# ydchen0806/CLC

Measured on AMD Instinct MI355X. Metric: images/sec fwd+bwd @256x256 bs8; bpp+PSNR parity vs ref, higher is better.
Workload: dtype f32; 1 GPU; CLC N=64 lambda=0.0067 MSE, 256x256 bs8/GPU, n_refs=1: fwd + RD loss + bwd + clip_grad_norm + AdamW + aux step (configs[1]); global_batch=8, parallelism=dp1, ranks_seen=1, collective=none, hip_graph=True

## Files before the change

### clc_amd/csrc/conv_wgrad.hip

```cpp
#include "common.h"

#include <type_traits>

namespace {

constexpr int BK = 32;

constexpr unsigned kOOB = 0x80000000u;

__device__ __forceinline__ f32x4 buf_load4(__amdgpu_buffer_rsrc_t rsrc, unsigned byte_off) {
  return __builtin_bit_cast(f32x4, __builtin_amdgcn_raw_buffer_load_b128(rsrc, byte_off, 0, 0));
}

__device__ __forceinline__ int pin_s(int x) {
  int r;
  asm("s_mov_b32 %0, %1" : "=s"(r) : "s"(x));
  return r;
}

__device__ __forceinline__ void dma16(__amdgpu_buffer_rsrc_t rsrc, float* lds_dst, unsigned byte_off) {
#if defined(__HIP_DEVICE_COMPILE__)
  __builtin_amdgcn_raw_ptr_buffer_load_lds(rsrc, (__attribute__((address_space(3))) void*)lds_dst, 16, byte_off, 0, 0, 0);
#endif
}

struct WgradParams {
  const float* x; const float* dy; float* partial; float* bias_partial;
  unsigned x_bytes, dy_bytes;
  const float* dys; int lddys, dys_act, dys_pre; unsigned dys_bytes;
  int ow_shift, img_shift;
  int rmw;
  int N, H, W, Cin, ldx;
  int OH, OW, Cout, lddy;
  int ks, stride, pad, in_op;
  int K;
  int k_per_split;
  int nci;
};

struct OutSpec { float* w; float* b; int mode; };
typedef __bf16 bf16x8 __attribute__((ext_vector_type(8)));
__device__ __forceinline__ void split3(const float (&v)[8], bf16x8& h, bf16x8& m, bf16x8& l) {
#pragma unroll
  for (int e = 0; e < 8; ++e) {
    const __bf16 hb = (__bf16)v[e];
    const float r = v[e] - (float)hb;
    const __bf16 mb = (__bf16)r;
    const float r2 = r - (float)mb;
    h[e] = hb; m[e] = mb; l[e] = (__bf16)r2;
  }
}
#define MFMA_BF(a, b, c) __builtin_amdgcn_mfma_f32_32x32x16_bf16((a), (b), (c), 0, 0, 0)
#define MFMA_SPLIT6(ah, am, al, bh, bm, bl, c) do { \
    c = MFMA_BF(al, bh, c); c = MFMA_BF(ah, bl, c); c = MFMA_BF(am, bm, c); \
    c = MFMA_BF(am, bh, c); c = MFMA_BF(ah, bm, c); c = MFMA_BF(ah, bh, c); } while (0)

template <int BM, int BN, int WM, int WN, bool DMA = false, int BF = 0>
__device__ __forceinline__ void wgrad_body(const WgradParams& p, const int bx, const int by, const int k_begin, const int k_end, const OutSpec o, const int tid) {
  constexpr int NT = 64 * WM * WN;
  constexpr int TM = BM / WM / 32, TN = BN / WN / 32;
  constexpr int A_P = (BK * BM / 4 + NT - 1) / NT, B_P = (BK * BN / 4 + NT - 1) / NT;
  constexpr int AQ = BM / 4, BQ = BN / 4;
  extern __shared__ __attribute__((aligned(16))) float smem[];
  float* As = smem;
  float* Bs = smem + 2 * BK * BM;

  const int lane = tid & 63, wave = tid >> 6;
  const int wm = wave / WN, wn = wave % WN;
  const int tap = bx / p.nci, ci0 = (bx % p.nci) * BN;
  const int kh = tap / p.ks, kw = tap - kh * p.ks;
  const int co0 = by * BM;
  const int ntiles = (k_end - k_begin + BK - 1) / BK;
  const bool do_bias = (o.b != nullptr) && (bx == 0);
  const int pCout = pin_s(p.Cout), pCin = pin_s(p.Cin), pH = pin_s(p.H), pW = pin_s(p.W), pOH = pin_s(p.OH), pOW = pin_s(p.OW);
  const int plddy = pin_s(p.lddy), plddys = pin_s(p.lddys), pldx = pin_s(p.ldx), pstride = pin_s(p.stride), ppad = pin_s(p.pad);
  const int pows = pin_s(p.ow_shift), pimgs = pin_s(p.img_shift), pact = pin_s(p.dys_act), ppre = pin_s(p.dys_pre);

  f32x4 a_reg[A_P], b_reg[B_P], bias_acc[A_P], s_reg[A_P];
#pragma unroll
  for (int i = 0; i < A_P; ++i) bias_acc[i] = (f32x4){0.f, 0.f, 0.f, 0.f};

  const __amdgpu_buffer_rsrc_t xr = __builtin_amdgcn_make_buffer_rsrc(const_cast<float*>(p.x), 0, p.x_bytes, 0x00020000);
  const __amdgpu_buffer_rsrc_t dr = __builtin_amdgcn_make_buffer_rsrc(const_cast<float*>(p.dy), 0, p.dy_bytes, 0x00020000);
  const bool sq = p.in_op == CLC_IN_SQUARE;
  const bool fuse_act = p.dys != nullptr;
  const __amdgpu_buffer_rsrc_t sr = __builtin_amdgcn_make_buffer_rsrc(const_cast<float*>(fuse_act ? p.dys : p.dy), 0, fuse_act ? p.dys_bytes : p.dy_bytes, 0x00020000);
  auto load_tile = [&](int kt) {
    const int kbase = k_begin + kt * BK;
#pragma unroll
    for (int i = 0; i < A_P; ++i) {
      const int piece = tid + i * NT, row = piece / AQ, q = piece - row * AQ;
      const int pix = kbase + row, co = co0 + q * 4;
      const bool ok = row < BK && pix < k_end && co < pCout;
      a_reg[i] = buf_load4(dr, ok ? ((unsigned)pix * (unsigned)plddy + (unsigned)co) * 4u : kOOB);
      if (fuse_act) s_reg[i] = buf_load4(sr, ok ? ((unsigned)pix * (unsigned)plddys + (unsigned)co) * 4u : kOOB);
    }
#pragma unroll
    for (int i = 0; i < B_P; ++i) {
      const int piece = tid + i * NT, row = piece / BQ, q = piece - row * BQ;
      const int pix = kbase + row, ci = ci0 + q * 4;
      const int pp = pix < k_end ? pix : k_begin;
      int n, oy, ox;
      if (pows >= 0) {
        n = pp >> pimgs;
        const int r = pp & ((1 << pimgs) - 1);
        oy = r >> pows; ox = r & ((1 << pows) - 1);
      } else {
        n = pp / (pOH * pOW);
        const int r = pp - n * (pOH * pOW);
        oy = r / pOW; ox = r - oy * pOW;
      }
      const int iy = oy * pstride - ppad + kh, ix = ox * pstride - ppad + kw;
      const bool ok = row < BK && pix < k_end && ci < pCin && (unsigned)iy < (unsigned)pH && (unsigned)ix < (unsigned)pW;
      b_reg[i] = buf_load4(xr, ok ? ((unsigned)((n * pH + iy) * pW + ix) * (unsigned)pldx + (unsigned)ci) * 4u : kOOB);
    }
  };
  static_assert(!DMA || ((BK * BM / 4) % NT == 0 && (BK * BN / 4) % NT == 0), "whole DMA instructions per tile");
  constexpr bool use_dma = DMA;
  const int wave_base = (tid >> 6) * 64;
  auto dma_tile = [&](int kt, int buf) {
    const int kbase = k_begin + kt * BK;
#pragma unroll
    for (int i = 0; i < A_P; ++i) {
      const int piece = tid + i * NT, row = piece / AQ, q = piece - row * AQ;
      const int pix = kbase + row, co = co0 + q * 4;
      const bool ok = pix < k_end && co < pCout;
      dma16(dr, As + buf * BK * BM + (i * NT + wave_base) * 4, ok ? ((unsigned)pix * (unsigned)plddy + (unsigned)co) * 4u : kOOB);
    }
#pragma unroll
    for (int i = 0; i < B_P; ++i) {
      const int piece = tid + i * NT, row = piece / BQ, q = piece - row * BQ;
      const int pix = kbase + row, ci = ci0 + q * 4;
      const int pp = pix < k_end ? pix : k_begin;
      int n, oy, ox;
      if (pows >= 0) {
        n = pp >> pimgs;
        const int r = pp & ((1 << pimgs) - 1);
        oy = r >> pows; ox = r & ((1 << pows) - 1);
      } else {
        n = pp / (pOH * pOW);
        const int r = pp - n * (pOH * pOW);
// ... 537 lines not shown
  long unit_end[kMaxGroup];
  int T[kMaxGroup];
  int gx[kMaxGroup], gy[kMaxGroup];
  float* slots;
  int* plan;
  WgradParams p[kMaxGroup];
};

struct SKSeg { int idx, tile, k0, k1; };
__device__ __forceinline__ int sk_tid() {
  int t = threadIdx.x;
  asm volatile("" : "+v"(t));
  return t;
}
__device__ __forceinline__ int sk_find(const SKGroup& g, long u, int lo) {
  int hi = g.count - 1;
  while (lo < hi) {
    const int mid = (lo + hi) >> 1;
    if (u >= g.unit_end[mid]) lo = mid + 1; else hi = mid;
  }
  return lo;
}
__device__ __forceinline__ SKSeg sk_locate(const SKGroup& g, long u, long end, int& idx) {
  idx = sk_find(g, u, idx);
  const long base = idx ? g.unit_end[idx - 1] : 0;
  const int T = g.T[idx];
  const long local = u - base;
  SKSeg sgm;
  sgm.idx = idx;
  sgm.tile = (int)(local / T);
  sgm.k0 = (int)(local - (long)sgm.tile * T);
  const long k1 = (long)sgm.k0 + (end - u);
  sgm.k1 = k1 < T ? (int)k1 : T;
  return sgm;
}
__device__ __forceinline__ void sk_write_plan(const SKGroup& g, int w, long u0, long end) {
  if (threadIdx.x != 0) return;
  int idx = 0;
  const SKSeg sgm = sk_locate(g, u0, end, idx);
  int e0 = 0, e1 = 0, e2 = 0, e3 = 0;
  if (sgm.k0 > 0 && sgm.k1 == g.T[sgm.idx]) {
    const long ts = u0 - sgm.k0;
    long wf = ts * g.G / g.total;
    while ((wf + 1) * g.total / g.G <= ts) ++wf;
    while (wf * g.total / g.G > ts) --wf;
    e0 = sgm.idx; e1 = sgm.tile; e2 = (int)wf; e3 = 1;
  }
  int* dst = g.plan + 4 * w;
  dst[0] = e0; dst[1] = e1; dst[2] = e2; dst[3] = e3;
}

__device__ __forceinline__ OutSpec sk_out(const SKGroup& g, const WgradParams& p, const SKSeg& sgm, int T, int w, int tile_floats) {
  OutSpec o;
  if (sgm.k0 == 0 && sgm.k1 == T) {
    o.w = p.partial; o.b = p.bias_partial; o.mode = p.rmw ? 1 : 0;
  } else {
    float* slot = g.slots + ((size_t)w * 2 + (sgm.k0 > 0 ? 0 : 1)) * g.slot_floats;
    o.w = slot; o.b = p.bias_partial ? slot + tile_floats : nullptr; o.mode = 2;
  }
  return o;
}

template <int TW, bool DMA, int BF = 0>
__global__ __launch_bounds__(256, 2)
void conv_wgrad_taps_sk_kernel(const SKGroup g) {
  const int w = blockIdx.x;
  long u = (long)w * g.total / g.G;
  const long end = (long)(w + 1) * g.total / g.G;
  sk_write_plan(g, w, u, end);
  int idx = 0;
  bool first = true;
#pragma clang loop unroll(disable)
  while (u < end) {
    const SKSeg sgm = sk_locate(g, u, end, idx);
    const WgradParams& p = g.p[sgm.idx];
    const int gx = g.gx[sgm.idx];
    if (!first) __syncthreads();
    wgrad_taps_body<TW, DMA, BF>(p, sgm.tile % gx, sgm.tile / gx, sgm.k0, sgm.k1, sk_out(g, p, sgm, g.T[sgm.idx], w, 64 * 9 * 64), sk_tid());
    first = false;
    u += sgm.k1 - sgm.k0;
  }
}

constexpr int sk_wg_per_cu(int bm, int bn) { return bm * bn >= 128 * 128 ? 2 : (bm * bn >= 128 * 64 ? 3 : 5); }

template <int BM, int BN, int WM, int WN, bool DMA, int BF = 0>
__global__ __launch_bounds__(64 * WM * WN, (BM * BN >= 128 * 128 ? 2 : (BM * BN >= 128 * 64 ? 4 : 6)))
void conv_wgrad_sk_kernel(const SKGroup g) {
  const int w = blockIdx.x;
  long u = (long)w * g.total / g.G;
  const long end = (long)(w + 1) * g.total / g.G;
  sk_write_plan(g, w, u, end);
  int idx = 0;
  bool first = true;
#pragma clang loop unroll(disable)
  while (u < end) {
    const SKSeg sgm = sk_locate(g, u, end, idx);
    const WgradParams& p = g.p[sgm.idx];
    const int gx = g.gx[sgm.idx];
    if (!first) __syncthreads();
    const int ke = sgm.k1 * BK;
    wgrad_body<BM, BN, WM, WN, DMA, BF>(p, sgm.tile % gx, sgm.tile / gx, sgm.k0 * BK, ke < p.K ? ke : p.K, sk_out(g, p, sgm, g.T[sgm.idx], w, BM * BN), sk_tid());
    first = false;
    u += sgm.k1 - sgm.k0;
  }
}

constexpr int kFixY = 64;
template <int BM, int BN, int TAPS>
__global__ __launch_bounds__(256) void wgrad_sk_fixup_kernel(const SKGroup g) {
  constexpr int TILE = BM * TAPS * BN;
  __shared__ f32x4 sm[4][64];
  __shared__ int list[1280];
  __shared__ int wave_cnt[4];
  const int tid = threadIdx.x;
  int n_list = 0;
  {
    const int lane = tid & 63, wv = tid >> 6;
    for (int base = 0; base < g.G; base += 256) {
      const int w = base + tid;
      const bool on = w < g.G && g.plan[4 * w + 3] != 0;
      const unsigned long long m = __ballot(on);
      if (lane == 0) wave_cnt[wv] = __popcll(m);
      __syncthreads();
      int off = n_list, tot = 0;
      for (int q = 0; q < 4; ++q) { if (q < wv) off += wave_cnt[q]; tot += wave_cnt[q]; }
      if (on) list[off + __popcll(m & ((1ull << lane) - 1ull))] = w;
      n_list += tot;
      __syncthreads();
    }
  }
  const int col = tid & 63, grp = tid >> 6;
  const int e = (blockIdx.x * 64 + col) * 4;
  for (int li = blockIdx.y; li < n_list; li += kFixY) {
    const int wl = list[li];
    const int idx = g.plan[4 * wl], tile = g.plan[4 * wl + 1], wf = g.plan[4 * wl + 2];
    const WgradParams& p = g.p[idx];
    const int gx = g.gx[idx];
    const int bx = tile % gx, by = tile / gx;
    const bool is_bias = e >= TILE;
    const bool live = e < TILE + BM && !(is_bias && !(p.bias_partial && bx == 0));
    f32x4 s = {0.f, 0.f, 0.f, 0.f};
    if (live) {
      const int n = wl - wf + 1;
      auto src = [&](int i) { return reinterpret_cast<const f32x4*>(g.slots + ((size_t)(wf + i) * 2 + (i == 0 ? 1 : 0)) * g.slot_floats + e); };
      int i = grp;
      for (; i + 12 < n; i += 16) {
        const f32x4 a0 = *src(i), a1 = *src(i + 4), a2 = *src(i + 8), a3 = *src(i + 12);
        s += a0; s += a1; s += a2; s += a3;
      }
      for (; i < n; i += 4) s += *src(i);
    }
    __syncthreads();
    sm[grp][col] = s;
    __syncthreads();
    if (grp != 0 || !live) continue;
    s = (sm[0][col] + sm[1][col]) + (sm[2][col] + sm[3][col]);
    const int co0 = by * BM;
    if (is_bias) {
      const int c = e - TILE;
#pragma unroll
      for (int q = 0; q < 4; ++q)
        if (co0 + c + q < p.Cout) { float* dst = p.bias_partial + co0 + c + q; *dst = (p.rmw ? *dst : 0.f) + s[q]; }
      continue;
    }
    int cl, tap, cil, ci0, T9;
    if (TAPS == 9) { cl = e / (9 * BN); const int r = e - cl * 9 * BN; tap = r / BN; cil = r - tap * BN; ci0 = bx * BN; T9 = 9; }
    else { cl = e / BN; cil = e - cl * BN; tap = bx / p.nci; ci0 = (bx - tap * p.nci) * BN; T9 = p.ks * p.ks; }
    const int co = co0 + cl, ci = ci0 + cil;
    if (co >= p.Cout || ci >= p.Cin) continue;
    f32x4* dst = reinterpret_cast<f32x4*>(p.partial + ((size_t)co * T9 + tap) * p.Cin + ci);
// ... 65 lines not shown
      const int k = e >> 7, c = e & 127, pix = kb + k;
      float gv = (pix < k_end && co0 + c < p.Cout) ? p.dy[(size_t)pix * p.lddy + co0 + c] : 0.f;
      if (p.dys && pix < k_end && co0 + c < p.Cout) gv *= act_deriv(p.dys[(size_t)pix * p.lddys + co0 + c], p.dys_act, p.dys_pre);
      dyS[k][c] = gv;
    }
    for (int e = tid; e < 32 * 32; e += 256) {
      const int k = e >> 5, j = e & 31, pix = kb + k;
      float v = 0.f;
      if (pix < k_end && j < ncol) {
        const int tap = j / p.Cin, ci = j - tap * p.Cin, kh = tap / p.ks, kw = tap - kh * p.ks;
        const int n = pix / (p.OH * p.OW), r = pix - n * (p.OH * p.OW);
        const int oy = r / p.OW, ox = r - oy * p.OW;
        const int iy = oy * p.stride - p.pad + kh, ix = ox * p.stride - p.pad + kw;
        if (iy >= 0 && ix >= 0 && iy < p.H && ix < p.W) {
          v = p.x[(size_t)((n * p.H + iy) * p.W + ix) * p.ldx + ci];
          if (p.in_op == CLC_IN_SQUARE) v *= v;
        }
      }
      xS[k][j] = v;
    }
    __syncthreads();
#pragma unroll 4
    for (int k = 0; k < 32; ++k) {
      const float g = dyS[k][co_l];
      bsum += g;
#pragma unroll
      for (int j = 0; j < 16; ++j) acc[j] = fmaf(g, xS[k][jh * 16 + j], acc[j]);
    }
  }
  if (co < p.Cout) {
#pragma unroll
    for (int j = 0; j < 16; ++j)
      if (jh * 16 + j < ncol) {
        float* dst = p.partial + ((size_t)split * p.Cout + co) * ncol + jh * 16 + j;
        *dst = p.rmw ? *dst + acc[j] : acc[j];
      }
    if (jh == 0 && p.bias_partial) {
      float* dst = p.bias_partial + (size_t)split * p.Cout + co;
      *dst = p.rmw ? *dst + bsum : bsum;
    }
  }
}

struct Plan { int bm, bn, splits, k_per_split, nci; bool small; int taps; };

Plan make_plan(const clc_wgrad_desc* d) {
  Plan pl;
  pl.taps = 0;
  const long K = (long)d->N * d->OH * d->OW;
  const int T = d->ks * d->ks;
  pl.small = !((d->Cin % 4 == 0) && (d->ldx % 4 == 0) && (d->Cout % 4 == 0) && (d->lddy % 4 == 0));
  if (pl.small) {
    pl.bm = pl.bn = 0; pl.nci = 1;
    int splits = (int)((K + 255) / 256);
    if (splits < 1) splits = 1;
    if (splits > 512) splits = 512;
    long kps = (K + splits - 1) / splits;
    pl.k_per_split = (int)kps; pl.splits = (int)((K + kps - 1) / kps);
    return pl;
  }
  {
    auto lg = [](int v) { int s = 0; while ((1 << s) < v) ++s; return (1 << s) == v ? s : -1; };
    const int la = lg(d->OW), lb = lg(d->OH * d->OW), tw = d->OW < 32 ? d->OW : 32;
    const bool eligible = d->ks == 3 && d->stride == 1 && d->pad == 1 && la >= 3 && lb >= 0 && d->OH >= 32 / tw;
    if (eligible) {
      pl.taps = tw; pl.bm = 64; pl.bn = 64; pl.nci = (d->Cin + 63) / 64;
      const long ktiles = K / 32, tiles = (long)((d->Cout + 63) / 64) * pl.nci;
      long sp = (ktiles + 15) / 16;
      const long fill = (256 + tiles - 1) / tiles;
      if (sp < fill) sp = fill;
      if (sp > ktiles / 2) sp = ktiles / 2 > 0 ? ktiles / 2 : 1;
      const long cap = 512 / tiles > 0 ? 512 / tiles : 1;
      if (sp > cap) sp = cap;
      const long kt = (ktiles + sp - 1) / sp;
      pl.k_per_split = (int)(kt * 32);
      pl.splits = (int)((ktiles + kt - 1) / kt);
      return pl;
    }
  }
  const int bms[2] = {128, 64}, bns[2] = {128, 64};
  const long wsz = (long)d->Cout * T * d->Cin;
  long best_cost = -1, splits = 1;
  pl.bm = 64; pl.bn = 64;
  for (int a = 0; a < 2; ++a)
    for (int b = 0; b < 2; ++b) {
      const int bm = bms[a], bn = bns[b];
      if (bm == 128 && d->Cout < 128) continue;
      if (bn == 128 && (d->Cin < 128 || d->Cin % 128 != 0)) continue;
      const long tiles = (long)((d->Cout + bm - 1) / bm) * ((d->Cin + bn - 1) / bn) * T;
      const long eff_pct = (bm == 128 && bn == 128) ? 100 : ((bm == 128 || bn == 128) ? 80 : 55);
      const long mfma_per_ktile = (long)(bm / 32) * (bn / 32) / 4 * 16 * 64 * 100 / eff_pct;
      const long max_sp = K / 64 > 0 ? K / 64 : 1;
      for (long sp = 1; sp <= 256 && sp <= max_sp; ++sp) {
        const long ktiles = (K / sp + BK - 1) / BK;
        const long chain = ktiles * mfma_per_ktile + 6000;
        const long rounds = (tiles * sp + 255) / 256;
        const long slab = sp > 1 ? 12000 + sp * wsz / 200 : 0;
        const long cost = rounds * chain + slab;
        if (best_cost < 0 || cost < best_cost) { best_cost = cost; pl.bm = bm; pl.bn = bn; splits = sp; }
      }
    }
  pl.nci = (d->Cin + pl.bn - 1) / pl.bn;
  long kps = (K + splits - 1) / splits;
  kps = (kps + BK - 1) / BK * BK;
  pl.k_per_split = (int)kps;
  pl.splits = (int)((K + kps - 1) / kps);
  return pl;
}

}

extern "C" size_t clc_conv2d_wgrad_workspace_bytes(const clc_wgrad_desc* d) {
  if (!d) return 0;
  if (d->ks == 5) return clc_conv5_wgrad_workspace_bytes(d);
  Plan pl = make_plan(d);
  const size_t wsz = (size_t)d->Cout * d->ks * d->ks * d->Cin;
  return ((size_t)pl.splits * (wsz + d->Cout) + 64) * sizeof(float);
}

namespace {

int prepare(const clc_wgrad_desc* d, Plan& pl, WgradParams& p, bool sk = false) {
  CLC_CHECK(d && d->x && d->dy && d->dw, "clc_conv2d_wgrad: null pointer");
  CLC_CHECK(d->ks == 1 || d->ks == 3, "clc_conv2d_wgrad: ks must be 1 or 3 here (ks = 5 problems are launched in line by clc_conv2d_wgrad, never grouped)");
  CLC_CHECK(d->stride == 1 || d->stride == 2, "clc_conv2d_wgrad: stride must be 1 or 2");
  CLC_CHECK(d->OH == (d->H + 2 * d->pad - d->ks) / d->stride + 1 && d->OW == (d->W + 2 * d->pad - d->ks) / d->stride + 1,
            "clc_conv2d_wgrad: output dims inconsistent");
  CLC_CHECK(d->ldx >= d->Cin && d->lddy >= d->Cout, "clc_conv2d_wgrad: ld too small");
  CLC_CHECK((long)d->N * d->H * d->W < (1l << 31) && (long)d->N * d->OH * d->OW < (1l << 31), "clc_conv2d_wgrad: too many pixels");
  pl = make_plan(d);
  if (!(sk && clc_tuning[CLC_TUNE_WGRAD_STREAMK] && !pl.small))
    CLC_CHECK(d->workspace && d->workspace_bytes >= clc_conv2d_wgrad_workspace_bytes(d), "clc_conv2d_wgrad: workspace too small");
  const int T = d->ks * d->ks;
  const size_t wsz = (size_t)d->Cout * T * d->Cin;
  p.x = d->x; p.dy = d->dy;
  const bool direct = (pl.splits == 1);
  p.rmw = direct && d->accumulate;
  p.partial = direct ? d->dw : (float*)d->workspace;
  p.bias_partial = d->dbias ? (direct ? d->dbias : (float*)d->workspace + (size_t)pl.splits * wsz) : nullptr;
  p.N = d->N; p.H = d->H; p.W = d->W; p.Cin = d->Cin; p.ldx = d->ldx;
  p.OH = d->OH; p.OW = d->OW; p.Cout = d->Cout; p.lddy = d->lddy;
  p.ks = d->ks; p.stride = d->stride; p.pad = d->pad; p.in_op = d->in_op;
  p.K = d->N * d->OH * d->OW; p.k_per_split = pl.k_per_split; p.nci = pl.nci;
  const size_t xb = ((size_t)d->N * d->H * d->W - 1) * d->ldx * 4 + (size_t)d->Cin * 4;
  const size_t db = ((size_t)d->N * d->OH * d->OW - 1) * d->lddy * 4 + (size_t)d->Cout * 4;
  CLC_CHECK(xb < (1ull << 31) && db < (1ull << 31), "clc_conv2d_wgrad: tensor larger than 2 GiB");
  p.x_bytes = (unsigned)xb; p.dy_bytes = (unsigned)db;
  auto lg = [](int v) { int s = 0; while ((1 << s) < v) ++s; return (1 << s) == v ? s : -1; };
  const int la = lg(d->OW), lb = lg(d->OH * d->OW);
  p.ow_shift = (la >= 0 && lb >= 0) ? la : -1; p.img_shift = (la >= 0 && lb >= 0) ? lb : -1;
  p.dys = d->dys; p.lddys = d->lddys; p.dys_act = d->dys_act; p.dys_pre = d->dys_pre; p.dys_bytes = 0;
  if (d->dys) {
    CLC_CHECK(d->lddys >= d->Cout, "clc_conv2d_wgrad: bad dys");
    const size_t sb = ((size_t)d->N * d->OH * d->OW - 1) * d->lddys * 4 + (size_t)d->Cout * 4;
    CLC_CHECK(sb < (1ull << 31), "clc_conv2d_wgrad: dys larger than 2 GiB");
    p.dys_bytes = (unsigned)sb;
  }
  if (pl.small) CLC_CHECK(T * d->Cin <= 32, "clc_conv2d_wgrad: small/unaligned path needs ks*ks*Cin <= 32 (got %d)", T * d->Cin);
  else CLC_CHECK(aligned16(d->x) && aligned16(d->dy), "clc_conv2d_wgrad: unaligned pointers");
  return 0;
}

struct Pending { const clc_wgrad_desc* d; Plan pl; WgradParams p; };

template <int BM, int BN>
int launch_variant(const Pending* pend, int n, hipStream_t st) {
  WgradGroup g;
  g.count = 0;
  int total = 0;
  for (int i = 0; i < n; ++i) {
    const Pending& e = pend[i];
    if (e.pl.small || e.pl.taps || e.pl.bm != BM || e.pl.bn != BN) continue;
    const int T = e.d->ks * e.d->ks;
    const int gx = e.pl.nci * T, gy = (e.d->Cout + BM - 1) / BM;
    total += gx * gy * e.pl.splits;
    g.gx[g.count] = gx; g.gy[g.count] = gy; g.wg_end[g.count] = total; g.p[g.count] = e.p;
    ++g.count;
  }
  if (g.count == 0) return 0;
  const size_t lds = (size_t)2 * BK * (BM + BN) * sizeof(float);
  if (g.count == 1) {
    const int last = g.wg_end[0] / (g.gx[0] * g.gy[0]);
    hipLaunchKernelGGL((conv_wgrad_kernel<BM, BN, 2, 2>), dim3(g.gx[0], g.gy[0], last), dim3(256), lds, st, g.p[0]);
  } else {
    hipLaunchKernelGGL((conv_wgrad_grouped_kernel<BM, BN, 2, 2>), dim3(total), dim3(256), lds, st, g);
  }
  CLC_LAUNCH_CHECK();
  return 0;
}

template <int TW>
int launch_taps(const Pending* pend, int n, hipStream_t st) {
  WgradGroup g;
  g.count = 0;
  int total = 0;
  for (int i = 0; i < n; ++i) {
    const Pending& e = pend[i];
    if (e.pl.small || e.pl.taps != TW) continue;
    const int gx = e.pl.nci, gy = (e.d->Cout + 63) / 64;
    total += gx * gy * e.pl.splits;
    g.gx[g.count] = gx; g.gy[g.count] = gy; g.wg_end[g.count] = total; g.p[g.count] = e.p;
    ++g.count;
  }
  if (g.count == 0) return 0;
  constexpr int XP = (32 / TW + 2) * (TW + 2);
  const size_t lds = (size_t)2 * (32 * 64 + XP * 64) * sizeof(float);
  static PerDeviceOnce attr_once;
  if (attr_once.first()) {
    (void)hipFuncSetAttribute(reinterpret_cast<const void*>(&conv_wgrad_taps_kernel<TW>), hipFuncAttributeMaxDynamicSharedMemorySize, (int)lds);
    (void)hipFuncSetAttribute(reinterpret_cast<const void*>(&conv_wgrad_taps_grouped_kernel<TW>), hipFuncAttributeMaxDynamicSharedMemorySize, (int)lds);
  }
  if (g.count == 1) {
    const int last = g.wg_end[0] / (g.gx[0] * g.gy[0]);
    hipLaunchKernelGGL((conv_wgrad_taps_kernel<TW>), dim3(g.gx[0], g.gy[0], last), dim3(256), lds, st, g.p[0]);
  } else {
    hipLaunchKernelGGL((conv_wgrad_taps_grouped_kernel<TW>), dim3(total), dim3(256), lds, st, g);
  }
  CLC_LAUNCH_CHECK();
  return 0;
}

int flush(Pending* pend, int& n, hipStream_t st) {
  if (n == 0) return 0;
  for (int i = 0; i < n; ++i)
    if (pend[i].pl.small) {
      hipLaunchKernelGGL(wgrad_small_kernel, dim3(pend[i].pl.splits, (pend[i].d->Cout + 127) / 128), dim3(256), 0, st, pend[i].p, pend[i].pl.splits);
      CLC_LAUNCH_CHECK();
    }
  int rc;
  if ((rc = launch_variant<128, 128>(pend, n, st)) < 0) return rc;
  if ((rc = launch_variant<128, 64>(pend, n, st)) < 0) return rc;
  if ((rc = launch_variant<64, 128>(pend, n, st)) < 0) return rc;
  if ((rc = launch_variant<64, 64>(pend, n, st)) < 0) return rc;
  if ((rc = launch_taps<32>(pend, n, st)) < 0) return rc;
  if ((rc = launch_taps<16>(pend, n, st)) < 0) return rc;
  if ((rc = launch_taps<8>(pend, n, st)) < 0) return rc;
  SlabGroup sg;
  sg.count = 0;
  int blocks = 0;
  for (int i = 0; i < n; ++i) {
    const Pending& e = pend[i];
    if (e.pl.splits == 1) continue;
    const long wsz = (long)e.d->Cout * e.d->ks * e.d->ks * e.d->Cin;
    blocks += (int)((wsz + 255) / 256);
    sg.e[sg.count] = SlabSet{e.p.partial, e.d->dw, wsz, e.pl.splits, e.d->accumulate};
    sg.blk_end[sg.count++] = blocks;
    if (e.d->dbias) {
      blocks += (e.d->Cout + 255) / 256;
      sg.e[sg.count] = SlabSet{e.p.bias_partial, e.d->dbias, (long)e.d->Cout, e.pl.splits, e.d->accumulate};
      sg.blk_end[sg.count++] = blocks;
    }
  }
  if (sg.count) {
    hipLaunchKernelGGL(slab_reduce_kernel, dim3(blocks), dim3(256), 0, st, sg);
    CLC_LAUNCH_CHECK();
  }
  n = 0;
  return 0;
}

constexpr int kCUs = 256;
constexpr size_t sk_slot_floats(int tile_floats, int bm) { return (size_t)((tile_floats + bm + 255) / 256 * 256); }
constexpr size_t kSKPlanFloats = 4 * 1280 + 1536;
constexpr size_t kSKRegion[7] = {
    (size_t)kCUs * sk_wg_per_cu(128, 128) * 2 * sk_slot_floats(128 * 128, 128), (size_t)kCUs * sk_wg_per_cu(128, 64) * 2 * sk_slot_floats(128 * 64, 128),
    (size_t)kCUs * sk_wg_per_cu(64, 128) * 2 * sk_slot_floats(64 * 128, 64),    (size_t)kCUs * sk_wg_per_cu(64, 64) * 2 * sk_slot_floats(64 * 64, 64),
    (size_t)kCUs * 2 * 2 * sk_slot_floats(64 * 9 * 64, 64), (size_t)kCUs * 2 * 2 * sk_slot_floats(64 * 9 * 64, 64),
    (size_t)kCUs * 2 * 2 * sk_slot_floats(64 * 9 * 64, 64)};
constexpr size_t sk_total_floats() { size_t t = 0; for (int i = 0; i < 7; ++i) t += kSKRegion[i] + kSKPlanFloats; return t; }

template <typename Pred, typename Geo>
bool sk_collect(const Pending* pend, int n, SKGroup& g, float* region, int slot_floats, int max_g, int min_units, Pred pred, Geo geo) {
  g.count = 0; g.total = 0; g.plan = reinterpret_cast<int*>(region); g.slots = region + kSKPlanFloats; g.slot_floats = slot_floats;
  for (int i = 0; i < n; ++i) {
    const Pending& e = pend[i];
    if (e.pl.small || !pred(e)) continue;
    int gx, gy, T;
    geo(e, gx, gy, T);
    g.gx[g.count] = gx; g.gy[g.count] = gy; g.T[g.count] = T;
    g.total += (long)gx * gy * T;
    g.unit_end[g.count] = g.total;
    g.p[g.count] = e.p;
    g.p[g.count].partial = e.d->dw;
    g.p[g.count].bias_partial = e.d->dbias;
    g.p[g.count].rmw = e.d->accumulate;
    ++g.count;
  }
  if (g.count == 0) return false;
  long G = g.total / min_units;
  g.G = (int)(G < 1 ? 1 : (G > max_g ? max_g : G));
  return true;
}

inline bool dma_ok(const Pending& e) { return clc_tuning[CLC_TUNE_WGRAD_DMA] && e.d->dys == nullptr && e.d->in_op == CLC_IN_NONE; }
inline int bf_ok(const Pending& e) {
  if (!dma_ok(e)) return 0;
  if (clc_tuning[CLC_TUNE_BF16] && (long)e.d->OH * e.d->OW > 256) return 1;
  if (!e.pl.taps && e.pl.bm == 64 && e.pl.bn == 64) return 0;
  return (clc_tuning[CLC_TUNE_SPLIT] & (e.pl.taps ? 1 : 2)) ? 2 : 0;
}

template <int BM, int BN, bool DMA, int BF = 0>
int launch_variant_sk(const Pending* pend, int n, float* region, hipStream_t st) {
  static thread_local SKGroup g;
  constexpr int slot = (int)sk_slot_floats(BM * BN, BM);
  if (!sk_collect(pend, n, g, region, slot, kCUs * sk_wg_per_cu(BM, BN), 16, [](const Pending& e) { return !e.pl.taps && e.pl.bm == BM && e.pl.bn == BN && dma_ok(e) == DMA && bf_ok(e) == BF; },
                  [](const Pending& e, int& gx, int& gy, int& T) {
                    gx = e.pl.nci * e.d->ks * e.d->ks; gy = (e.d->Cout + BM - 1) / BM; T = (e.p.K + BK - 1) / BK;
                  })) return 0;
  const size_t lds = (size_t)2 * BK * (BM + BN) * sizeof(float);
  hipLaunchKernelGGL((conv_wgrad_sk_kernel<BM, BN, 2, 2, DMA, BF>), dim3(g.G), dim3(256), lds, st, g);
  CLC_LAUNCH_CHECK();
  if (g.G > 1) {
    hipLaunchKernelGGL((wgrad_sk_fixup_kernel<BM, BN, 1>), dim3((BM * BN + BM + 255) / 256, kFixY), dim3(256), 0, st, g);
    CLC_LAUNCH_CHECK();
  }
  return 0;
}

template <int TW, bool DMA, int BF = 0>
int launch_taps_sk(const Pending* pend, int n, float* region, hipStream_t st) {
  static thread_local SKGroup g;
  constexpr int slot = (int)sk_slot_floats(64 * 9 * 64, 64);
  if (!sk_collect(pend, n, g, region, slot, kCUs * 2, 4, [](const Pending& e) { return e.pl.taps == TW && dma_ok(e) == DMA && bf_ok(e) == BF; },
                  [](const Pending& e, int& gx, int& gy, int& T) { gx = e.pl.nci; gy = (e.d->Cout + 63) / 64; T = e.p.K >> 5; })) return 0;
  constexpr int XP = (32 / TW + 2) * (TW + 2);
  const size_t lds = (size_t)2 * (32 * 64 + XP * 64) * sizeof(float);
  static PerDeviceOnce attr_once;
  if (attr_once.first()) {
    (void)hipFuncSetAttribute(reinterpret_cast<const void*>(&conv_wgrad_taps_sk_kernel<TW, DMA, BF>), hipFuncAttributeMaxDynamicSharedMemorySize, (int)lds);
  }
  hipLaunchKernelGGL((conv_wgrad_taps_sk_kernel<TW, DMA, BF>), dim3(g.G), dim3(256), lds, st, g);
  CLC_LAUNCH_CHECK();
  if (g.G > 1) {
    hipLaunchKernelGGL((wgrad_sk_fixup_kernel<64, 64, 9>), dim3((64 * 9 * 64 + 64 + 255) / 256, kFixY), dim3(256), 0, st, g);
    CLC_LAUNCH_CHECK();
  }
  return 0;
}

int flush_sk(Pending* pend, int& n, float* ws, hipStream_t st) {
  if (n == 0) return 0;
  SlabGroup sg;
  sg.count = 0;
  int blocks = 0;
  for (int i = 0; i < n; ++i)
    if (pend[i].pl.small) {
      const Pending& e = pend[i];
      hipLaunchKernelGGL(wgrad_small_kernel, dim3(e.pl.splits, (e.d->Cout + 127) / 128), dim3(256), 0, st, e.p, e.pl.splits);
      CLC_LAUNCH_CHECK();
      if (e.pl.splits == 1) continue;
      const long wsz = (long)e.d->Cout * e.d->ks * e.d->ks * e.d->Cin;
      blocks += (int)((wsz + 255) / 256);
      sg.e[sg.count] = SlabSet{e.p.partial, e.d->dw, wsz, e.pl.splits, e.d->accumulate};
      sg.blk_end[sg.count++] = blocks;
      if (e.d->dbias) {
        blocks += (e.d->Cout + 255) / 256;
        sg.e[sg.count] = SlabSet{e.p.bias_partial, e.d->dbias, (long)e.d->Cout, e.pl.splits, e.d->accumulate};
        sg.blk_end[sg.count++] = blocks;
      }
    }
  if (sg.count) {
    hipLaunchKernelGGL(slab_reduce_kernel, dim3(blocks), dim3(256), 0, st, sg);
    CLC_LAUNCH_CHECK();
  }
  int rc;
  float* r = ws;
  if ((rc = launch_variant_sk<128, 128, true>(pend, n, r, st)) < 0) return rc;
  if ((rc = launch_variant_sk<128, 128, true, 1>(pend, n, r, st)) < 0) return rc;
  if ((rc = launch_variant_sk<128, 128, true, 2>(pend, n, r, st)) < 0) return rc;
  if ((rc = launch_variant_sk<128, 128, false>(pend, n, r, st)) < 0) return rc;
  r += kSKRegion[0] + kSKPlanFloats;
  if ((rc = launch_variant_sk<128, 64, true>(pend, n, r, st)) < 0) return rc;
  if ((rc = launch_variant_sk<128, 64, true, 1>(pend, n, r, st)) < 0) return rc;
  if ((rc = launch_variant_sk<128, 64, true, 2>(pend, n, r, st)) < 0) return rc;
  if ((rc = launch_variant_sk<128, 64, false>(pend, n, r, st)) < 0) return rc;
  r += kSKRegion[1] + kSKPlanFloats;
  if ((rc = launch_variant_sk<64, 128, true>(pend, n, r, st)) < 0) return rc;
  if ((rc = launch_variant_sk<64, 128, true, 1>(pend, n, r, st)) < 0) return rc;
  if ((rc = launch_variant_sk<64, 128, true, 2>(pend, n, r, st)) < 0) return rc;
  if ((rc = launch_variant_sk<64, 128, false>(pend, n, r, st)) < 0) return rc;
  r += kSKRegion[2] + kSKPlanFloats;
  if ((rc = launch_variant_sk<64, 64, true>(pend, n, r, st)) < 0) return rc;
  if ((rc = launch_variant_sk<64, 64, true, 1>(pend, n, r, st)) < 0) return rc;
  if ((rc = launch_variant_sk<64, 64, true, 2>(pend, n, r, st)) < 0) return rc;
  if ((rc = launch_variant_sk<64, 64, false>(pend, n, r, st)) < 0) return rc;
  r += kSKRegion[3] + kSKPlanFloats;
  if ((rc = launch_taps_sk<32, true>(pend, n, r, st)) < 0) return rc;
  if ((rc = launch_taps_sk<32, true, 1>(pend, n, r, st)) < 0) return rc;
  if ((rc = launch_taps_sk<32, true, 2>(pend, n, r, st)) < 0) return rc;
  if ((rc = launch_taps_sk<32, false>(pend, n, r, st)) < 0) return rc;
  r += kSKRegion[4] + kSKPlanFloats;
  if ((rc = launch_taps_sk<16, true>(pend, n, r, st)) < 0) return rc;
  if ((rc = launch_taps_sk<16, true, 1>(pend, n, r, st)) < 0) return rc;
  if ((rc = launch_taps_sk<16, true, 2>(pend, n, r, st)) < 0) return rc;
  if ((rc = launch_taps_sk<16, false>(pend, n, r, st)) < 0) return rc;
  r += kSKRegion[5] + kSKPlanFloats;
  if ((rc = launch_taps_sk<8, true>(pend, n, r, st)) < 0) return rc;
  if ((rc = launch_taps_sk<8, true, 1>(pend, n, r, st)) < 0) return rc;
  if ((rc = launch_taps_sk<8, true, 2>(pend, n, r, st)) < 0) return rc;
  if ((rc = launch_taps_sk<8, false>(pend, n, r, st)) < 0) return rc;
  n = 0;
  return 0;
}

int variant_id(const Plan& pl) { return pl.small ? 1 : (pl.taps ? 64900 + pl.taps : pl.bm * 1000 + pl.bn); }

}

extern "C" int clc_conv2d_wgrad(const clc_wgrad_desc* d, clc_stream_t stream) {
  if (d && d->ks == 5) return clc_conv5_wgrad_launch(d, (hipStream_t)stream);
  Pending e;
  e.d = d;
  int rc = prepare(d, e.pl, e.p);
  if (rc < 0) return rc;
  int n = 1;
  if ((rc = flush(&e, n, (hipStream_t)stream)) < 0) return rc;
  return variant_id(e.pl);
}

extern "C" int clc_conv2d_wgrad_batched(const clc_wgrad_desc* descs, int count, clc_stream_t stream) {
  CLC_CHECK(descs && count >= 0, "clc_conv2d_wgrad_batched: bad arguments");
  Pending pend[kMaxGroup];
  int n = 0, rc;
  for (int i = 0; i < count; ++i) {
    const clc_wgrad_desc* d = descs + i;
    bool clash = n == kMaxGroup;
    for (int j = 0; j < n && !clash; ++j)
      clash = pend[j].d->dw == d->dw || (d->dbias && pend[j].d->dbias == d->dbias) || pend[j].d->workspace == d->workspace;
    if (clash && (rc = flush(pend, n, (hipStream_t)stream)) < 0) return rc;
    pend[n].d = d;
    if ((rc = prepare(d, pend[n].pl, pend[n].p)) < 0) return rc;
    ++n;
  }
  return flush(pend, n, (hipStream_t)stream);
}

extern "C" int clc_conv2d_wgrad_variant(const clc_wgrad_desc* d) {
  if (!d) return -1;
  if (d->ks == 5) return 5;
  return variant_id(make_plan(d));
}

extern "C" size_t clc_conv2d_wgrad_group_workspace_bytes(void) { return sk_total_floats() * sizeof(float); }

extern "C" size_t clc_conv2d_wgrad_sk_workspace_bytes(const clc_wgrad_desc* d) {
  if (!d) return 0;
  if (d->ks == 5) return clc_conv5_wgrad_workspace_bytes(d);
  if (clc_tuning[CLC_TUNE_WGRAD_STREAMK] && !make_plan(d).small) return 0;
  return clc_conv2d_wgrad_workspace_bytes(d);
}

extern "C" int clc_conv2d_wgrad_batched_sk(const clc_wgrad_desc* descs, int count, void* group_workspace, size_t group_workspace_bytes,
                                          clc_stream_t stream) {
  CLC_CHECK(descs && count >= 0, "clc_conv2d_wgrad_batched_sk: bad arguments");
  CLC_CHECK(group_workspace && group_workspace_bytes >= clc_conv2d_wgrad_group_workspace_bytes() && aligned16(group_workspace),
            "clc_conv2d_wgrad_batched_sk: group workspace too small / unaligned");
  if (!clc_tuning[CLC_TUNE_WGRAD_STREAMK]) return clc_conv2d_wgrad_batched(descs, count, stream);
  Pending pend[kMaxGroup];
  int n = 0, rc;
  for (int i = 0; i < count; ++i) {
    const clc_wgrad_desc* d = descs + i;
    bool clash = n == kMaxGroup;
    for (int j = 0; j < n && !clash; ++j)
      clash = pend[j].d->dw == d->dw || (d->dbias && pend[j].d->dbias == d->dbias) || (d->workspace && pend[j].d->workspace == d->workspace);
    if (clash && (rc = flush_sk(pend, n, (float*)group_workspace, (hipStream_t)stream)) < 0) return rc;
    pend[n].d = d;
    if ((rc = prepare(d, pend[n].pl, pend[n].p, true)) < 0) return rc;
    ++n;
  }
  return flush_sk(pend, n, (float*)group_workspace, (hipStream_t)stream);
}
```

### clc_amd/csrc/rans_host.cpp

```cpp
#include <cmath>
#include <cstdint>
#include <cstdio>
#include <cstdlib>
#include <cstring>
#include <new>
#include <stdarg.h>
#include <vector>

#include "../../include/clc_hip.h"

static thread_local char g_err[512] = "";
void clc_set_error(const char* fmt, ...) {
  va_list ap;
  va_start(ap, fmt);
  vsnprintf(g_err, sizeof(g_err), fmt, ap);
  va_end(ap);
}
extern "C" const char* clc_last_error(void) { return g_err; }
extern "C" int clc_version(void) { return 200; }

#define CLC_TUNING_DEFAULTS {2, 1, 1, 0, 1024, 64, 1, 8, 1, 1, 1, 1, 0, 1, 0, 1, 3, 1, 1, 1, 1, 1, 1, 7, 3}
int clc_tuning[25] = CLC_TUNING_DEFAULTS;
static const int clc_tuning_default[25] = CLC_TUNING_DEFAULTS;
static bool clc_tuning_retired(int key) { return key == 0 || key == 2 || key == 3 || key == 12 || key == 19; }
extern "C" int clc_set_tuning(int key, int value) {
  if (key < 0 || key >= (int)(sizeof(clc_tuning) / sizeof(clc_tuning[0]))) { clc_set_error("clc_set_tuning: key %d out of range", key); return -1; }
  if (clc_tuning_retired(key) && value != clc_tuning_default[key]) {
    clc_set_error("clc_set_tuning: key %d is retired; it only accepts its last default, %d (got %d)", key, clc_tuning_default[key], value);
    return -1;
  }
  const int old = clc_tuning[key];
  clc_tuning[key] = value;
  return old;
}
extern "C" int clc_get_tuning(int key) {
  if (key < 0 || key >= (int)(sizeof(clc_tuning) / sizeof(clc_tuning[0]))) { clc_set_error("clc_get_tuning: key %d out of range", key); return -1; }
  return clc_tuning[key];
}
static uint32_t clc_order_hash(bool* dflt_out) {
  const int kGeneration = 6;
  static const int order_keys[] = {0, 4, 5, 12, 14, 16};
  uint32_t h = 2166136261u ^ (uint32_t)kGeneration;
  bool dflt = true;
  for (int k : order_keys) {
    int v = clc_tuning[k], d = clc_tuning_default[k];
    if (k == 16) { v &= 5; d &= 5; }
    if (v != d) dflt = false;
    h = (h ^ (uint32_t)v) * 16777619u;
  }
  if (dflt_out) *dflt_out = dflt;
  return h;
}
extern "C" int clc_kernel_config_tag(void) {
  const int kGeneration = 6;
  bool dflt = true;
  const uint32_t h = clc_order_hash(&dflt);
  return dflt ? kGeneration : (int)(128u | (h & 127u));
}
extern "C" unsigned clc_kernel_config_hash(void) { return clc_order_hash(nullptr); }

namespace {
constexpr int kPrec = 16, kBypassBits = 4;
constexpr uint32_t kBypassMax = (1u << kBypassBits) - 1;
constexpr uint64_t kL = 1ull << 31;

struct BackWriter {
  uint32_t* begin;
  uint32_t* ptr;
  bool overflow = false;
  inline void put(uint32_t w) {
    if (ptr == begin) { overflow = true; return; }
    *--ptr = w;
  }
};

inline void enc_put(uint64_t& x, BackWriter& o, uint32_t start, uint32_t freq) {
  const uint64_t x_max = ((kL >> kPrec) << 32) * freq;
  if (x >= x_max) { o.put((uint32_t)x); x >>= 32; }
  x = ((x / freq) << kPrec) + (x % freq) + start;
}
inline void enc_put_bits(uint64_t& x, BackWriter& o, uint32_t val) {
  const uint64_t x_max = ((kL >> 16) << 32) * (uint64_t)(1u << (16 - kBypassBits));
  if (x >= x_max) { o.put((uint32_t)x); x >>= 32; }
  x = (x << kBypassBits) | val;
}
}

extern "C" long clc_rans_encode_bound(long n) { return 4 * (n * 12 + 18); }

extern "C" long clc_rans_encode(const int32_t* symbols, const int32_t* indexes, long n, const int32_t* cdfs, int cdf_stride,
                                const int32_t* cdf_sizes, const int32_t* offsets, uint8_t* out, long out_cap) {
  if (n < 0 || (n > 0 && (!symbols || !indexes)) || !cdfs || !cdf_sizes || !offsets || !out) { clc_set_error("clc_rans_encode: bad args"); return -1; }
  if (out_cap < 8 || (reinterpret_cast<uintptr_t>(out) & 3)) { clc_set_error("clc_rans_encode: output buffer too small or unaligned"); return -1; }
  BackWriter o;
  o.begin = reinterpret_cast<uint32_t*>(out);
  o.ptr = o.begin + out_cap / 4;
  uint32_t* const end = o.ptr;
  uint64_t x = kL;
  for (long i = n - 1; i >= 0; --i) {
    const int32_t ci = indexes[i];
    const int32_t* cdf = cdfs + (long)ci * cdf_stride;
    const int32_t max_value = cdf_sizes[ci] - 2;
    if (max_value < 0 || cdf_sizes[ci] > cdf_stride) { clc_set_error("clc_rans_encode: bad cdf size at index %d", ci); return -1; }
    int32_t value = symbols[i] - offsets[ci];
// ... 117 lines not shown
```

Measured before the change: 341.3 images/sec.

## Add whole-filter wgrad tiles for small 1x1 convs with BK16 K-tiles

Adds wide wgrad tile shapes (256x64, 64x256, 192x64) that cover the entire Cout x Cin filter of small 1x1 convolutions in one tile, with a smaller K-tile of 16 pixels to keep LDS use in bounds. This applies both to the direct and stream-K paths, with extra workspace regions and an opt-in for more dynamic shared memory. The aim is to read each input and grad-output pixel once instead of once per output tile. The path is enabled by default through a new bit in the wgrad DMA tuning key. It risks lower occupancy and more K-tile loop overhead from the halved BK.

```diff
diff --git a/clc_amd/csrc/conv_wgrad.hip b/clc_amd/csrc/conv_wgrad.hip
--- a/clc_amd/csrc/conv_wgrad.hip
+++ b/clc_amd/csrc/conv_wgrad.hip
@@ -5,6 +5,15 @@
 namespace {
 
 constexpr int BK = 32;
+
+#ifndef CLC_WGRAD_WHOLE_BK
+#define CLC_WGRAD_WHOLE_BK 16
+#endif
+constexpr int kWholeBK = CLC_WGRAD_WHOLE_BK;
+static_assert(kWholeBK == 16 || kWholeBK == 32, "K-tile of the whole-filter shapes: 16 or 32 pixels");
+constexpr bool wide_tile(int bm, int bn) { return bm > 128 || bn > 128; }
+constexpr int tile_bk(int bm, int bn) { return wide_tile(bm, bn) ? kWholeBK : BK; }
+constexpr bool whole_shape(int cout, int cin) { return cout > 0 && cin > 0 && cout % 64 == 0 && cin % 64 == 0 && cout * cin <= 16384 && cin != 192; }
 
 constexpr unsigned kOOB = 0x80000000u;
 
@@ -57,6 +66,7 @@
 
 template <int BM, int BN, int WM, int WN, bool DMA = false, int BF = 0>
 __device__ __forceinline__ void wgrad_body(const WgradParams& p, const int bx, const int by, const int k_begin, const int k_end, const OutSpec o, const int tid) {
+  constexpr int BK = tile_bk(BM, BN);
   constexpr int NT = 64 * WM * WN;
   constexpr int TM = BM / WM / 32, TN = BN / WN / 32;
   constexpr int A_P = (BK * BM / 4 + NT - 1) / NT, B_P = (BK * BN / 4 + NT - 1) / NT;
@@ -760,11 +770,12 @@
   }
 }
 
-constexpr int sk_wg_per_cu(int bm, int bn) { return bm * bn >= 128 * 128 ? 2 : (bm * bn >= 128 * 64 ? 3 : 5); }
+constexpr int sk_wg_per_cu(int bm, int bn) { return wide_tile(bm, bn) ? (kWholeBK == 16 ? 3 : 2) : (bm * bn >= 128 * 128 ? 2 : (bm * bn >= 128 * 64 ? 3 : 5)); }
 
 template <int BM, int BN, int WM, int WN, bool DMA, int BF = 0>
-__global__ __launch_bounds__(64 * WM * WN, (BM * BN >= 128 * 128 ? 2 : (BM * BN >= 128 * 64 ? 4 : 6)))
+__global__ __launch_bounds__(64 * WM * WN, (wide_tile(BM, BN) ? sk_wg_per_cu(BM, BN) : (BM * BN >= 128 * 128 ? 2 : (BM * BN >= 128 * 64 ? 4 : 6))))
 void conv_wgrad_sk_kernel(const SKGroup g) {
+  constexpr int BK = tile_bk(BM, BN);
   const int w = blockIdx.x;
   long u = (long)w * g.total / g.G;
   const long end = (long)(w + 1) * g.total / g.G;
@@ -996,13 +1007,15 @@
   const long wsz = (long)d->Cout * T * d->Cin;
   long best_cost = -1, splits = 1;
   pl.bm = 64; pl.bn = 64;
+  const bool whole = (clc_tuning[CLC_TUNE_WGRAD_DMA] & 2) && d->ks == 1 && whole_shape(d->Cout, d->Cin);
   for (int a = 0; a < 2; ++a)
     for (int b = 0; b < 2; ++b) {
-      const int bm = bms[a], bn = bns[b];
-      if (bm == 128 && d->Cout < 128) continue;
-      if (bn == 128 && (d->Cin < 128 || d->Cin % 128 != 0)) continue;
+      const int bm = whole ? d->Cout : bms[a], bn = whole ? d->Cin : bns[b];
+      if (whole && (a || b)) continue;
+      if (!whole && bm == 128 && d->Cout < 128) continue;
+      if (!whole && bn == 128 && (d->Cin < 128 || d->Cin % 128 != 0)) continue;
       const long tiles = (long)((d->Cout + bm - 1) / bm) * ((d->Cin + bn - 1) / bn) * T;
-      const long eff_pct = (bm == 128 && bn == 128) ? 100 : ((bm == 128 || bn == 128) ? 80 : 55);
+      const long eff_pct = bm * bn >= 128 * 128 ? 100 : (bm * bn >= 128 * 64 ? 80 : 55);
       const long mfma_per_ktile = (long)(bm / 32) * (bn / 32) / 4 * 16 * 64 * 100 / eff_pct;
       const long max_sp = K / 64 > 0 ? K / 64 : 1;
       for (long sp = 1; sp <= 256 && sp <= max_sp; ++sp) {
@@ -1092,7 +1105,14 @@
     ++g.count;
   }
   if (g.count == 0) return 0;
-  const size_t lds = (size_t)2 * BK * (BM + BN) * sizeof(float);
+  constexpr size_t lds = (size_t)2 * tile_bk(BM, BN) * (BM + BN) * sizeof(float);
+  if constexpr (lds > 65536) {
+    static PerDeviceOnce attr_once;
+    if (attr_once.first()) {
+      (void)hipFuncSetAttribute(reinterpret_cast<const void*>(&conv_wgrad_kernel<BM, BN, 2, 2>), hipFuncAttributeMaxDynamicSharedMemorySize, (int)lds);
+      (void)hipFuncSetAttribute(reinterpret_cast<const void*>(&conv_wgrad_grouped_kernel<BM, BN, 2, 2>), hipFuncAttributeMaxDynamicSharedMemorySize, (int)lds);
+    }
+  }
   if (g.count == 1) {
     const int last = g.wg_end[0] / (g.gx[0] * g.gy[0]);
     hipLaunchKernelGGL((conv_wgrad_kernel<BM, BN, 2, 2>), dim3(g.gx[0], g.gy[0], last), dim3(256), lds, st, g.p[0]);
@@ -1142,6 +1162,9 @@
       CLC_LAUNCH_CHECK();
     }
   int rc;
+  if ((rc = launch_variant<256, 64>(pend, n, st)) < 0) return rc;
+  if ((rc = launch_variant<64, 256>(pend, n, st)) < 0) return rc;
+  if ((rc = launch_variant<192, 64>(pend, n, st)) < 0) return rc;
   if ((rc = launch_variant<128, 128>(pend, n, st)) < 0) return rc;
   if ((rc = launch_variant<128, 64>(pend, n, st)) < 0) return rc;
   if ((rc = launch_variant<64, 128>(pend, n, st)) < 0) return rc;
@@ -1176,12 +1199,15 @@
 constexpr int kCUs = 256;
 constexpr size_t sk_slot_floats(int tile_floats, int bm) { return (size_t)((tile_floats + bm + 255) / 256 * 256); }
 constexpr size_t kSKPlanFloats = 4 * 1280 + 1536;
-constexpr size_t kSKRegion[7] = {
+constexpr int kSKRegions = 10;
+constexpr size_t kSKRegion[kSKRegions] = {
     (size_t)kCUs * sk_wg_per_cu(128, 128) * 2 * sk_slot_floats(128 * 128, 128), (size_t)kCUs * sk_wg_per_cu(128, 64) * 2 * sk_slot_floats(128 * 64, 128),
     (size_t)kCUs * sk_wg_per_cu(64, 128) * 2 * sk_slot_floats(64 * 128, 64),    (size_t)kCUs * sk_wg_per_cu(64, 64) * 2 * sk_slot_floats(64 * 64, 64),
     (size_t)kCUs * 2 * 2 * sk_slot_floats(64 * 9 * 64, 64), (size_t)kCUs * 2 * 2 * sk_slot_floats(64 * 9 * 64, 64),
-    (size_t)kCUs * 2 * 2 * sk_slot_floats(64 * 9 * 64, 64)};
-constexpr size_t sk_total_floats() { size_t t = 0; for (int i = 0; i < 7; ++i) t += kSKRegion[i] + kSKPlanFloats; return t; }
+    (size_t)kCUs * 2 * 2 * sk_slot_floats(64 * 9 * 64, 64),
+    (size_t)kCUs * sk_wg_per_cu(256, 64) * 2 * sk_slot_floats(256 * 64, 256), (size_t)kCUs * sk_wg_per_cu(64, 256) * 2 * sk_slot_floats(64 * 256, 64),
+    (size_t)kCUs * sk_wg_per_cu(192, 64) * 2 * sk_slot_floats(192 * 64, 192)};
+constexpr size_t sk_total_floats() { size_t t = 0; for (int i = 0; i < kSKRegions; ++i) t += kSKRegion[i] + kSKPlanFloats; return t; }
 
 template <typename Pred, typename Geo>
 bool sk_collect(const Pending* pend, int n, SKGroup& g, float* region, int slot_floats, int max_g, int min_units, Pred pred, Geo geo) {
@@ -1206,7 +1232,7 @@
   return true;
 }
 
-inline bool dma_ok(const Pending& e) { return clc_tuning[CLC_TUNE_WGRAD_DMA] && e.d->dys == nullptr && e.d->in_op == CLC_IN_NONE; }
+inline bool dma_ok(const Pending& e) { return (clc_tuning[CLC_TUNE_WGRAD_DMA] & 1) && e.d->dys == nullptr && e.d->in_op == CLC_IN_NONE; }
 inline int bf_ok(const Pending& e) {
   if (!dma_ok(e)) return 0;
   if (clc_tuning[CLC_TUNE_BF16] && (long)e.d->OH * e.d->OW > 256) return 1;
@@ -1218,11 +1244,16 @@
 int launch_variant_sk(const Pending* pend, int n, float* region, hipStream_t st) {
   static thread_local SKGroup g;
   constexpr int slot = (int)sk_slot_floats(BM * BN, BM);
+  constexpr int KB = tile_bk(BM, BN);
   if (!sk_collect(pend, n, g, region, slot, kCUs * sk_wg_per_cu(BM, BN), 16, [](const Pending& e) { return !e.pl.taps && e.pl.bm == BM && e.pl.bn == BN && dma_ok(e) == DMA && bf_ok(e) == BF; },
                   [](const Pending& e, int& gx, int& gy, int& T) {
-                    gx = e.pl.nci * e.d->ks * e.d->ks; gy = (e.d->Cout + BM - 1) / BM; T = (e.p.K + BK - 1) / BK;
+                    gx = e.pl.nci * e.d->ks * e.d->ks; gy = (e.d->Cout + BM - 1) / BM; T = (e.p.K + KB - 1) / KB;
                   })) return 0;
-  const size_t lds = (size_t)2 * BK * (BM + BN) * sizeof(float);
+  constexpr size_t lds = (size_t)2 * KB * (BM + BN) * sizeof(float);
+  if constexpr (lds > 65536) {
+    static PerDeviceOnce attr_once;
+    if (attr_once.first()) (void)hipFuncSetAttribute(reinterpret_cast<const void*>(&conv_wgrad_sk_kernel<BM, BN, 2, 2, DMA, BF>), hipFuncAttributeMaxDynamicSharedMemorySize, (int)lds);
+  }
   hipLaunchKernelGGL((conv_wgrad_sk_kernel<BM, BN, 2, 2, DMA, BF>), dim3(g.G), dim3(256), lds, st, g);
   CLC_LAUNCH_CHECK();
   if (g.G > 1) {
@@ -1314,6 +1345,21 @@
   if ((rc = launch_taps_sk<8, true, 1>(pend, n, r, st)) < 0) return rc;
   if ((rc = launch_taps_sk<8, true, 2>(pend, n, r, st)) < 0) return rc;
   if ((rc = launch_taps_sk<8, false>(pend, n, r, st)) < 0) return rc;
+  r += kSKRegion[6] + kSKPlanFloats;
+  if ((rc = launch_variant_sk<256, 64, true>(pend, n, r, st)) < 0) return rc;
+  if ((rc = launch_variant_sk<256, 64, true, 1>(pend, n, r, st)) < 0) return rc;
+  if ((rc = launch_variant_sk<256, 64, true, 2>(pend, n, r, st)) < 0) return rc;
+  if ((rc = launch_variant_sk<256, 64, false>(pend, n, r, st)) < 0) return rc;
+  r += kSKRegion[7] + kSKPlanFloats;
+  if ((rc = launch_variant_sk<64, 256, true>(pend, n, r, st)) < 0) return rc;
+  if ((rc = launch_variant_sk<64, 256, true, 1>(pend, n, r, st)) < 0) return rc;
+  if ((rc = launch_variant_sk<64, 256, true, 2>(pend, n, r, st)) < 0) return rc;
+  if ((rc = launch_variant_sk<64, 256, false>(pend, n, r, st)) < 0) return rc;
+  r += kSKRegion[8] + kSKPlanFloats;
+  if ((rc = launch_variant_sk<192, 64, true>(pend, n, r, st)) < 0) return rc;
+  if ((rc = launch_variant_sk<192, 64, true, 1>(pend, n, r, st)) < 0) return rc;
+  if ((rc = launch_variant_sk<192, 64, true, 2>(pend, n, r, st)) < 0) return rc;
+  if ((rc = launch_variant_sk<192, 64, false>(pend, n, r, st)) < 0) return rc;
   n = 0;
   return 0;
 }
diff --git a/clc_amd/csrc/rans_host.cpp b/clc_amd/csrc/rans_host.cpp
--- a/clc_amd/csrc/rans_host.cpp
+++ b/clc_amd/csrc/rans_host.cpp
@@ -19,7 +19,7 @@
 extern "C" const char* clc_last_error(void) { return g_err; }
 extern "C" int clc_version(void) { return 200; }
 
-#define CLC_TUNING_DEFAULTS {2, 1, 1, 0, 1024, 64, 1, 8, 1, 1, 1, 1, 0, 1, 0, 1, 3, 1, 1, 1, 1, 1, 1, 7, 3}
+#define CLC_TUNING_DEFAULTS {2, 1, 1, 0, 1024, 64, 1, 8, 1, 3, 1, 1, 0, 1, 0, 1, 3, 1, 1, 1, 1, 1, 1, 7, 3}
 int clc_tuning[25] = CLC_TUNING_DEFAULTS;
 static const int clc_tuning_default[25] = CLC_TUNING_DEFAULTS;
 static bool clc_tuning_retired(int key) { return key == 0 || key == 2 || key == 3 || key == 12 || key == 19; }
```

After: 342.4 images/sec, median of 6. About the same (+0.3%).
